# tqch/ddpm-torch

Hardware: AMD Instinct MI355X
Metric: training imgs/s/GPU + 1000-step DDPM samples/s, CIFAR-10 UNet @1/2/4/8 MI355X (higher is better)
Workload: dtype bf16; 1 GPU; configs/cifar10.json UNet (35.7M params), full Trainer.step, B=128 per GPU, 32x32, T=1000, dropout 0.1, Adam+clip+EMA; global_batch=128, rccl_ranks=1, parallelism=dp1

## Files before the change

### ddpm-torch_amd/csrc/common.h

```cpp
#pragma once
#include <hip/hip_runtime.h>
#include <stdint.h>

#define DDPM_OK 0
#define DDPM_ERR_SHAPE 1
#define DDPM_ERR_DTYPE 2
#define DDPM_ERR_ALIGN 3
#define DDPM_ERR_LAUNCH 4
#define DDPM_ERR_NULL 5

#define DDPM_F32 0
#define DDPM_BF16 1

typedef unsigned short bf16_t;

typedef float f32x4 __attribute__((ext_vector_type(4)));
typedef float f32x16 __attribute__((ext_vector_type(16)));
typedef short s16x8 __attribute__((ext_vector_type(8)));
typedef unsigned int u32x4 __attribute__((ext_vector_type(4)));

__device__ __forceinline__ float bf2f(bf16_t v) { return __uint_as_float(((unsigned)v) << 16); }
typedef __attribute__((ext_vector_type(2))) __bf16 hw_bf16x2;
typedef __attribute__((ext_vector_type(2))) float hw_f32x2;
__device__ __forceinline__ unsigned pack_bf2(float lo, float hi) {
    hw_f32x2 v; v.x = lo; v.y = hi;
    return __builtin_bit_cast(unsigned, __builtin_convertvector(v, hw_bf16x2));
}
__device__ __forceinline__ bf16_t f2bf(float f) { return (bf16_t)(pack_bf2(f, 0.f) & 0xffffu); }

template <typename T> struct Elem;
template <> struct Elem<float> {
    static constexpr int VEC = 4;
    __device__ static __forceinline__ float ld(const float* p) { return *p; }
    __device__ static __forceinline__ void st(float* p, float v) { *p = v; }
    __device__ static __forceinline__ void unpack(const u32x4& v, float* f) {
        f[0] = __uint_as_float(v.x); f[1] = __uint_as_float(v.y); f[2] = __uint_as_float(v.z); f[3] = __uint_as_float(v.w);
    }
    __device__ static __forceinline__ u32x4 pack(const float* f) {
        u32x4 v; v.x = __float_as_uint(f[0]); v.y = __float_as_uint(f[1]); v.z = __float_as_uint(f[2]); v.w = __float_as_uint(f[3]);
        return v;
    }
};
template <> struct Elem<bf16_t> {
    static constexpr int VEC = 8;
    __device__ static __forceinline__ float ld(const bf16_t* p) { return bf2f(*p); }
    __device__ static __forceinline__ void st(bf16_t* p, float v) { *p = f2bf(v); }
    __device__ static __forceinline__ void unpack(const u32x4& v, float* f) {
        f[0] = __uint_as_float(v.x << 16); f[1] = __uint_as_float(v.x & 0xffff0000u);
        f[2] = __uint_as_float(v.y << 16); f[3] = __uint_as_float(v.y & 0xffff0000u);
        f[4] = __uint_as_float(v.z << 16); f[5] = __uint_as_float(v.z & 0xffff0000u);
        f[6] = __uint_as_float(v.w << 16); f[7] = __uint_as_float(v.w & 0xffff0000u);
    }
    __device__ static __forceinline__ u32x4 pack(const float* f) {
        u32x4 v; v.x = pack_bf2(f[0], f[1]); v.y = pack_bf2(f[2], f[3]); v.z = pack_bf2(f[4], f[5]); v.w = pack_bf2(f[6], f[7]);
        return v;
    }
};

__device__ __forceinline__ u32x4 ldg16(const void* p) { return *reinterpret_cast<const u32x4*>(p); }
__device__ __forceinline__ void stg16(void* p, const u32x4& v) { *reinterpret_cast<u32x4*>(p) = v; }
__device__ __forceinline__ u32x4 zero16() { u32x4 v; v.x = v.y = v.z = v.w = 0u; return v; }

__device__ __forceinline__ float wave_sum(float v) {
#pragma unroll
    for (int o = 32; o > 0; o >>= 1) v += __shfl_xor(v, o, 64);
    return v;
}
__device__ __forceinline__ float wave_max(float v) {
#pragma unroll
    for (int o = 32; o > 0; o >>= 1) v = fmaxf(v, __shfl_xor(v, o, 64));
    return v;
}

__device__ __forceinline__ float sigmoidf_(float z) { return 1.0f / (1.0f + __expf(-z)); }
__device__ __forceinline__ float siluf_(float z) { return z * sigmoidf_(z); }
__device__ __forceinline__ float silu_fast_(float z) { return z * __builtin_amdgcn_rcpf(1.0f + __expf(-z)); }
__device__ __forceinline__ float silu_gradf_(float z) { float s = sigmoidf_(z); return s * (1.0f + z * (1.0f - s)); }

struct FastDiv {
    unsigned mul, shift, d;
};
__device__ __forceinline__ unsigned fdiv(unsigned n, const FastDiv& f) {
    return (unsigned)(((unsigned long long)n * f.mul) >> f.shift);
}
static inline FastDiv make_fastdiv(unsigned d) {
    FastDiv f; f.d = d ? d : 1; f.mul = 1u << 31; f.shift = 31;
    if (d <= 1) return f;
    unsigned l = 0; while ((1ull << l) < d) ++l;
    f.shift = 31 + l;
    if ((1ull << l) == d) return f;
    f.mul = (unsigned)((1ull << f.shift) / d + 1);
    return f;
}

__device__ __forceinline__ unsigned mix32(unsigned x) {
    x ^= x >> 16; x *= 0x7feb352dU; x ^= x >> 15; x *= 0x846ca68bU; x ^= x >> 16;
    return x;
}
__device__ __forceinline__ unsigned dropout_word(unsigned long long seed, unsigned long long pair) {
    const unsigned lo = (unsigned)pair, hi = (unsigned)(pair >> 32);
    return mix32(lo ^ mix32(hi + (unsigned)seed) ^ (unsigned)(seed >> 32) * 0x9E3779B9u);
}
__device__ __forceinline__ bool dropout_keep(unsigned long long seed, unsigned long long idx, unsigned thresh16) {
    const unsigned w = dropout_word(seed, idx >> 1);
    return ((idx & 1) ? (w >> 16) : (w & 0xffffu)) >= thresh16;
}
__device__ __forceinline__ unsigned dropout_h0(unsigned long long seed) {
    return mix32((unsigned)seed) ^ ((unsigned)(seed >> 32) * 0x9E3779B9u);
}
__device__ __forceinline__ unsigned dropout_word32(unsigned h0, unsigned pair) { return mix32(pair ^ h0); }
static inline unsigned dropout_thresh16(float p) {
    const double th = (double)p * 65536.0;
    return th <= 0 ? 0u : (th >= 65536.0 ? 65536u : (unsigned)(th + 0.5));
}
__device__ __forceinline__ float silu_grad_fast_(float z) {
    const float s = __builtin_amdgcn_rcpf(1.0f + __expf(-z));
    return s * (1.0f + z * (1.0f - s));
}

#include <atomic>
struct DevOnce {
    std::atomic<unsigned long long> mask{0};
    static unsigned long long bit() { int d = 0; (void)hipGetDevice(&d); return 1ull << (d & 63); }
    bool operator!() const { return !(mask.load(std::memory_order_acquire) & bit()); }
    DevOnce& operator=(bool) { mask.fetch_or(bit(), std::memory_order_release); return *this; }
};

static inline int check_launch() { return hipGetLastError() == hipSuccess ? DDPM_OK : DDPM_ERR_LAUNCH; }
static inline bool aligned16(const void* p) { return (((uintptr_t)p) & 15) == 0; }

int ddpm_sumsq_finish_launch(const float* partial, int n, float* total_sq, void* stream);
int ddpm_reserved_cus();
static inline int ddpm_cu_budget(int wanted) { const int left = 256 - ddpm_reserved_cus(); return wanted < left ? wanted : (left > 1 ? left : 1); }
int ddpm_pointwise_launch(const void* x, long long x_ld, const void* w, void* y, long long y_ld, const float* bias, const void* residual,
                          long long res_ld, int accumulate, int M, int N, int K, int dry, void* stream);
int ddpm_edgeconv_few_out_launch(const void* x, long long x_ld, const void* w, void* y, const float* bias, int B, int H, int W, int C, int N,
                                 int dry, void* stream);
int ddpm_edgeconv_few_in_launch(const void* x, long long x_ld, const void* w, void* y, long long y_ld, const float* bias, int B, int H, int W,
                                int C, int N, int dry, void* stream);
int ddpm_conv3x3_stream_launch(const void* x, long long x_ld, const void* w, void* y, long long y_ld, const float* bias, const float* rowbias,
                               long long rowbias_ld, const void* residual, long long res_ld, int accumulate, int B, int H, int W, int C, int N,
                               int upsample, int xcd, int dry, void* stream);
```

### ddpm-torch_amd/csrc/plan.hip

```cpp
#include "common.h"
#include "../../include/ddpm_hip.h"
#include "../../include/ddpm_hip_debug.h"

#include <cstring>
#include <mutex>
#include <type_traits>
#include <utility>
#include <vector>

namespace {

typedef unsigned long long word_t;

template <class T> inline T from_word(word_t w) {
    if constexpr (std::is_pointer<T>::value) {
        return reinterpret_cast<T>(static_cast<uintptr_t>(w));
    } else if constexpr (std::is_same<T, float>::value) {
        const unsigned u = static_cast<unsigned>(w);
        float f;
        std::memcpy(&f, &u, 4);
        return f;
    } else {
        return static_cast<T>(w);
    }
}

typedef int (*thunk_t)(const word_t*);

template <class... A, size_t... I> inline int invoke(int (*fn)(A...), const word_t* w, std::index_sequence<I...>) {
    return fn(from_word<A>(w[I])...);
}
template <class... A> constexpr int arity(int (*)(A...)) { return (int)sizeof...(A); }
template <class... A> inline int invoke_all(int (*fn)(A...), const word_t* w) { return invoke(fn, w, std::index_sequence_for<A...>{}); }

struct EntryPoint {
    const char* name;
    thunk_t thunk;
    int nargs;
};

#define EP(fn) {#fn, [](const word_t* w) -> int { return invoke_all(&fn, w); }, arity(&fn)}

}

extern "C" int ddpm_stream_order(void* waiter, void* signaller);
extern "C" int ddpm_fill_zero(void* p, long long bytes, void* stream);

namespace {

const EntryPoint kEntryPoints[] = {
    EP(ddpm_conv2d_nhwc), EP(ddpm_conv2d_wgrad_nhwc), EP(ddpm_conv3x3_wgrad_nhwc), EP(ddpm_conv3x3_wgrad_up_nhwc), EP(ddpm_conv1x1_wgrad_nhwc),
    EP(ddpm_wgrad_reduce), EP(ddpm_wgrad_unpack), EP(ddpm_wgrad_unpack_sumsq), EP(ddpm_gemm),
    EP(ddpm_attention_fwd), EP(ddpm_attention_fwd_lse), EP(ddpm_attention_bwd), EP(ddpm_groupnorm_silu_fwd),
    EP(ddpm_groupnorm_silu_bwd), EP(ddpm_timestep_embedding), EP(ddpm_nchw_to_nhwc), EP(ddpm_pack_weight), EP(ddpm_pack_weight_multi),
    EP(ddpm_q_sample), EP(ddpm_mse_fwd), EP(ddpm_mse_bwd), EP(ddpm_weighted_sum_f32), EP(ddpm_atb_f32), EP(ddpm_p_sample_step), EP(ddpm_vlb_terms), EP(ddpm_vlb_terms_bwd), EP(ddpm_gather_i64),
    EP(ddpm_add_i64), EP(ddpm_gather_rows_f32), EP(ddpm_silu_fwd), EP(ddpm_silu_bwd), EP(ddpm_colsum), EP(ddpm_upsample2x_bwd), EP(ddpm_resample2x_nhwc),
    EP(ddpm_add_rows), EP(ddpm_softmax_fwd), EP(ddpm_softmax_bwd), EP(ddpm_sumsq_accumulate), EP(ddpm_adam_ema_step), EP(ddpm_mt_grad_sumsq),
    EP(ddpm_mt_adam_ema), EP(ddpm_mt_gather_f32), EP(ddpm_mfma_probe), EP(ddpm_copy_probe), EP(ddpm_dropout_mask), EP(ddpm_stream_order), EP(ddpm_fill_zero),
    EP(ddpm_toy_time_table), EP(ddpm_toy_decoder_fwd), EP(ddpm_toy_decoder_bwd), EP(ddpm_toy_time_table_bwd),
    EP(ddpm_manifold_kth_f16), EP(ddpm_manifold_cover_f16),
};
constexpr int kNumEntryPoints = (int)(sizeof(kEntryPoints) / sizeof(kEntryPoints[0]));

struct Entry {
    thunk_t thunk;
    int first_word;
    int ep;
};

struct Plan {
    std::vector<Entry> entries;
    std::vector<word_t> words;
    std::vector<int> segment_end;
    int failed_index = -1;
    int failed_status = 0;
};

constexpr int kRing = 2048;
struct EventRing {
    hipEvent_t ev[kRing];
    unsigned next = 0;
    bool ready = false;
};
EventRing g_rings[64];
std::mutex g_ring_mutex;

}

extern "C" {

int ddpm_stream_order(void* waiter, void* signaller) {
    if (waiter == signaller) return DDPM_OK;
    int dev = 0;
    if (hipGetDevice(&dev) != hipSuccess) return DDPM_ERR_LAUNCH;
    EventRing& r = g_rings[dev & 63];
    hipEvent_t e;
    {
        std::lock_guard<std::mutex> lock(g_ring_mutex);
        if (!r.ready) {
            for (int i = 0; i < kRing; ++i)
                if (hipEventCreateWithFlags(&r.ev[i], hipEventDisableTiming) != hipSuccess) return DDPM_ERR_LAUNCH;
            r.ready = true;
        }
        e = r.ev[r.next++ % kRing];
    }
    if (hipEventRecord(e, (hipStream_t)signaller) != hipSuccess) return DDPM_ERR_LAUNCH;
    if (hipStreamWaitEvent((hipStream_t)waiter, e, 0) != hipSuccess) return DDPM_ERR_LAUNCH;
    return DDPM_OK;
}

int ddpm_fill_zero(void* p, long long bytes, void* stream) {
    if (bytes < 0) return DDPM_ERR_SHAPE;
    if (bytes == 0) return DDPM_OK;
    if (!p) return DDPM_ERR_NULL;
    return hipMemsetAsync(p, 0, (size_t)bytes, (hipStream_t)stream) == hipSuccess ? DDPM_OK : DDPM_ERR_LAUNCH;
}

void* ddpm_plan_create(void) { return new Plan(); }

int ddpm_plan_destroy(void* plan) {
    delete static_cast<Plan*>(plan);
    return DDPM_OK;
}

int ddpm_plan_append(void* plan, const char* entry, const unsigned long long* words, int n_words) {
    if (!plan || !entry || (!words && n_words > 0)) return -DDPM_ERR_NULL;
    Plan* p = static_cast<Plan*>(plan);
    for (int i = 0; i < kNumEntryPoints; ++i) {
        if (std::strcmp(kEntryPoints[i].name, entry) != 0) continue;
        if (kEntryPoints[i].nargs != n_words) return -DDPM_ERR_SHAPE;
        Entry e;
        e.thunk = kEntryPoints[i].thunk;
        e.first_word = (int)p->words.size();
        e.ep = i;
        p->words.insert(p->words.end(), words, words + n_words);
        p->entries.push_back(e);
        return (int)p->entries.size() - 1;
    }
    return -DDPM_ERR_SHAPE;
}

int ddpm_plan_cut(void* plan) {
    if (!plan) return -DDPM_ERR_NULL;
    Plan* p = static_cast<Plan*>(plan);
    p->segment_end.push_back((int)p->entries.size());
    return (int)p->segment_end.size() - 1;
}

int ddpm_plan_segments(void* plan) {
    if (!plan) return -DDPM_ERR_NULL;
    Plan* p = static_cast<Plan*>(plan);
    const int closed = (int)p->segment_end.size();
    const int last_end = closed ? p->segment_end.back() : 0;
    return closed + ((int)p->entries.size() > last_end ? 1 : 0);
}

int ddpm_plan_entries(void* plan) { return plan ? (int)static_cast<Plan*>(plan)->entries.size() : -DDPM_ERR_NULL; }

int ddpm_plan_run(void* plan, int segment) {
    if (!plan) return DDPM_ERR_NULL;
    Plan* p = static_cast<Plan*>(plan);
    const int closed = (int)p->segment_end.size();
    if (segment < 0 || segment > closed) return DDPM_ERR_SHAPE;
    const int first = segment ? p->segment_end[segment - 1] : 0;
    const int last = segment < closed ? p->segment_end[segment] : (int)p->entries.size();
    const word_t* words = p->words.data();
    const Entry* e = p->entries.data();
    for (int i = first; i < last; ++i) {
        const int rc = e[i].thunk(words + e[i].first_word);
        if (rc != DDPM_OK) {
            p->failed_index = i;
            p->failed_status = rc;
            return rc;
        }
    }
    return DDPM_OK;
}

const char* ddpm_plan_failed_entry(void* plan, int* index) {
    if (!plan) return nullptr;
    Plan* p = static_cast<Plan*>(plan);
    if (index) *index = p->failed_index;
    return p->failed_index < 0 ? nullptr : kEntryPoints[p->entries[p->failed_index].ep].name;
}

int ddpm_plan_entry_arity(const char* entry) {
    if (!entry) return -1;
    for (int i = 0; i < kNumEntryPoints; ++i)
        if (std::strcmp(kEntryPoints[i].name, entry) == 0) return kEntryPoints[i].nargs;
    return -1;
}

}
```

Baseline: 14160 imgs/s.

## Attach completion events to producer kernel launches and drop redundant stream waits

Adds a plan resolution pass that, for each cross-stream ordering entry, finds the last kernel launched on the signalling stream and marks it as producer. The producer's kernel is then launched with hipExtLaunchKernel carrying a stop event, so the waiter can call hipStreamWaitEvent on it directly instead of issuing a separate event record. Duplicate edges with no intervening work are skipped. This cuts host-side API calls and queue packets per step, at the cost of overriding hipLaunchKernelGGL globally and relying on the kernel's last argument being its stream.

Result: faster. 14360 imgs/s (median of 6 runs) (+1.4%).

```diff
diff --git a/ddpm-torch_amd/csrc/common.h b/ddpm-torch_amd/csrc/common.h
--- a/ddpm-torch_amd/csrc/common.h
+++ b/ddpm-torch_amd/csrc/common.h
@@ -1,5 +1,6 @@
 #pragma once
 #include <hip/hip_runtime.h>
+#include <hip/hip_ext.h>
 #include <stdint.h>
 
 #define DDPM_OK 0
@@ -126,6 +127,28 @@
     DevOnce& operator=(bool) { mask.fetch_or(bit(), std::memory_order_release); return *this; }
 };
 
+struct DdpmLaunchEdge {
+    hipStream_t stream = nullptr;
+    hipEvent_t event = nullptr;
+    bool armed = false;
+    bool attached = false;
+};
+extern thread_local DdpmLaunchEdge g_ddpm_launch_edge;
+
+template <class... P> static inline void ddpm_launch_with_event(DdpmLaunchEdge& edge, void (*kernel)(P...), dim3 grid, dim3 block, unsigned lds,
+                                                                hipStream_t st, P... formal) {
+    void* args[sizeof...(P) + 1] = {(void*)&formal..., nullptr};
+    if (hipExtLaunchKernel((const void*)kernel, grid, block, args, lds, st, nullptr, edge.event, 0) == hipSuccess) edge.attached = true;
+}
+template <class... P, class... A> static inline void ddpm_launch(void (*kernel)(P...), dim3 grid, dim3 block, unsigned lds, hipStream_t st, A&&... args) {
+    static_assert(sizeof...(P) == sizeof...(A), "kernel argument count");
+    DdpmLaunchEdge& edge = g_ddpm_launch_edge;
+    if (edge.armed && edge.stream == st) ddpm_launch_with_event<P...>(edge, kernel, grid, block, lds, st, static_cast<P>(args)...);
+    else kernel<<<grid, block, lds, st>>>(args...);
+}
+#undef hipLaunchKernelGGL
+#define hipLaunchKernelGGL(kernel, grid, block, lds, stream, ...) ddpm_launch(kernel, dim3(grid), dim3(block), (unsigned)(lds), stream, __VA_ARGS__)
+
 static inline int check_launch() { return hipGetLastError() == hipSuccess ? DDPM_OK : DDPM_ERR_LAUNCH; }
 static inline bool aligned16(const void* p) { return (((uintptr_t)p) & 15) == 0; }
 
diff --git a/ddpm-torch_amd/csrc/plan.hip b/ddpm-torch_amd/csrc/plan.hip
--- a/ddpm-torch_amd/csrc/plan.hip
+++ b/ddpm-torch_amd/csrc/plan.hip
@@ -33,13 +33,17 @@
 template <class... A> constexpr int arity(int (*)(A...)) { return (int)sizeof...(A); }
 template <class... A> inline int invoke_all(int (*fn)(A...), const word_t* w) { return invoke(fn, w, std::index_sequence_for<A...>{}); }
 
+enum EntryKind { EP_KERNELS, EP_ENQUEUES, EP_EDGE };
+
 struct EntryPoint {
     const char* name;
     thunk_t thunk;
     int nargs;
-};
-
-#define EP(fn) {#fn, [](const word_t* w) -> int { return invoke_all(&fn, w); }, arity(&fn)}
+    EntryKind kind;
+};
+
+#define EP(fn) {#fn, [](const word_t* w) -> int { return invoke_all(&fn, w); }, arity(&fn), EP_KERNELS}
+#define EP_AS(fn, kind) {#fn, [](const word_t* w) -> int { return invoke_all(&fn, w); }, arity(&fn), kind}
 
 }
 
@@ -56,22 +60,28 @@
     EP(ddpm_q_sample), EP(ddpm_mse_fwd), EP(ddpm_mse_bwd), EP(ddpm_weighted_sum_f32), EP(ddpm_atb_f32), EP(ddpm_p_sample_step), EP(ddpm_vlb_terms), EP(ddpm_vlb_terms_bwd), EP(ddpm_gather_i64),
     EP(ddpm_add_i64), EP(ddpm_gather_rows_f32), EP(ddpm_silu_fwd), EP(ddpm_silu_bwd), EP(ddpm_colsum), EP(ddpm_upsample2x_bwd), EP(ddpm_resample2x_nhwc),
     EP(ddpm_add_rows), EP(ddpm_softmax_fwd), EP(ddpm_softmax_bwd), EP(ddpm_sumsq_accumulate), EP(ddpm_adam_ema_step), EP(ddpm_mt_grad_sumsq),
-    EP(ddpm_mt_adam_ema), EP(ddpm_mt_gather_f32), EP(ddpm_mfma_probe), EP(ddpm_copy_probe), EP(ddpm_dropout_mask), EP(ddpm_stream_order), EP(ddpm_fill_zero),
+    EP(ddpm_mt_adam_ema), EP(ddpm_mt_gather_f32), EP(ddpm_mfma_probe), EP(ddpm_copy_probe), EP(ddpm_dropout_mask), EP_AS(ddpm_stream_order, EP_EDGE), EP_AS(ddpm_fill_zero, EP_ENQUEUES),
     EP(ddpm_toy_time_table), EP(ddpm_toy_decoder_fwd), EP(ddpm_toy_decoder_bwd), EP(ddpm_toy_time_table_bwd),
     EP(ddpm_manifold_kth_f16), EP(ddpm_manifold_cover_f16),
 };
 constexpr int kNumEntryPoints = (int)(sizeof(kEntryPoints) / sizeof(kEntryPoints[0]));
+
+enum Mode : unsigned char { RUN, PRODUCER, WAIT, RECORD, SKIP };
 
 struct Entry {
     thunk_t thunk;
     int first_word;
     int ep;
+    Mode mode = RUN;
+    int producer = -1;
 };
 
 struct Plan {
     std::vector<Entry> entries;
     std::vector<word_t> words;
     std::vector<int> segment_end;
+    std::vector<hipEvent_t> bound;
+    size_t resolved_entries = 0, resolved_cuts = 0;
     int failed_index = -1;
     int failed_status = 0;
 };
@@ -79,34 +89,76 @@
 constexpr int kRing = 2048;
 struct EventRing {
     hipEvent_t ev[kRing];
-    unsigned next = 0;
+    std::atomic<unsigned> next{0};
     bool ready = false;
 };
 EventRing g_rings[64];
 std::mutex g_ring_mutex;
 
-}
+EventRing* ring_of_device() {
+    int dev = 0;
+    if (hipGetDevice(&dev) != hipSuccess) return nullptr;
+    EventRing& r = g_rings[dev & 63];
+    std::lock_guard<std::mutex> lock(g_ring_mutex);
+    if (!r.ready) {
+        for (int i = 0; i < kRing; ++i)
+            if (hipEventCreateWithFlags(&r.ev[i], hipEventDisableTiming) != hipSuccess) return nullptr;
+        r.ready = true;
+    }
+    return &r;
+}
+inline hipEvent_t next_event(EventRing& r) { return r.ev[r.next.fetch_add(1, std::memory_order_relaxed) % kRing]; }
+
+inline int record_and_wait(EventRing& r, hipStream_t waiter, hipStream_t signaller) {
+    const hipEvent_t e = next_event(r);
+    if (hipEventRecord(e, signaller) != hipSuccess) return DDPM_ERR_LAUNCH;
+    if (hipStreamWaitEvent(waiter, e, 0) != hipSuccess) return DDPM_ERR_LAUNCH;
+    return DDPM_OK;
+}
+
+void resolve(Plan* p) {
+    const int n = (int)p->entries.size();
+    const word_t* words = p->words.data();
+    for (Entry& e : p->entries) { e.mode = RUN; e.producer = -1; }
+    size_t seg = 0;
+    int first = 0;
+    for (int i = 0; i < n; ++i) {
+        while (seg < p->segment_end.size() && p->segment_end[seg] <= i) first = p->segment_end[seg++];
+        Entry& e = p->entries[i];
+        if (kEntryPoints[e.ep].kind != EP_EDGE) continue;
+        const word_t waiter = words[e.first_word], signaller = words[e.first_word + 1];
+        if (waiter == signaller) continue;
+        e.mode = RECORD;
+        for (int j = i - 1; j >= first; --j) {
+            const Entry& q = p->entries[j];
+            const EntryPoint& ep = kEntryPoints[q.ep];
+            if (ep.kind == EP_EDGE) {
+                if (words[q.first_word] == waiter && words[q.first_word + 1] == signaller) { e.mode = SKIP; break; }
+                if (words[q.first_word] == signaller && words[q.first_word + 1] != signaller) break;
+                continue;
+            }
+            if (words[q.first_word + ep.nargs - 1] != signaller) continue;
+            if (ep.kind == EP_KERNELS) { e.mode = WAIT; e.producer = j; }
+            break;
+        }
+        if (e.mode == WAIT) p->entries[e.producer].mode = PRODUCER;
+    }
+    p->bound.assign(n, nullptr);
+    p->resolved_entries = p->entries.size();
+    p->resolved_cuts = p->segment_end.size();
+}
+
+}
+
+thread_local DdpmLaunchEdge g_ddpm_launch_edge;
 
 extern "C" {
 
 int ddpm_stream_order(void* waiter, void* signaller) {
     if (waiter == signaller) return DDPM_OK;
-    int dev = 0;
-    if (hipGetDevice(&dev) != hipSuccess) return DDPM_ERR_LAUNCH;
-    EventRing& r = g_rings[dev & 63];
-    hipEvent_t e;
-    {
-        std::lock_guard<std::mutex> lock(g_ring_mutex);
-        if (!r.ready) {
-            for (int i = 0; i < kRing; ++i)
-                if (hipEventCreateWithFlags(&r.ev[i], hipEventDisableTiming) != hipSuccess) return DDPM_ERR_LAUNCH;
-            r.ready = true;
-        }
-        e = r.ev[r.next++ % kRing];
-    }
-    if (hipEventRecord(e, (hipStream_t)signaller) != hipSuccess) return DDPM_ERR_LAUNCH;
-    if (hipStreamWaitEvent((hipStream_t)waiter, e, 0) != hipSuccess) return DDPM_ERR_LAUNCH;
-    return DDPM_OK;
+    EventRing* r = ring_of_device();
+    if (!r) return DDPM_ERR_LAUNCH;
+    return record_and_wait(*r, (hipStream_t)waiter, (hipStream_t)signaller);
 }
 
 int ddpm_fill_zero(void* p, long long bytes, void* stream) {
@@ -164,10 +216,35 @@
     if (segment < 0 || segment > closed) return DDPM_ERR_SHAPE;
     const int first = segment ? p->segment_end[segment - 1] : 0;
     const int last = segment < closed ? p->segment_end[segment] : (int)p->entries.size();
+    if (p->resolved_entries != p->entries.size() || p->resolved_cuts != p->segment_end.size()) resolve(p);
     const word_t* words = p->words.data();
     const Entry* e = p->entries.data();
+    EventRing* ring = nullptr;
+    DdpmLaunchEdge& arm = g_ddpm_launch_edge;
     for (int i = first; i < last; ++i) {
-        const int rc = e[i].thunk(words + e[i].first_word);
+        const word_t* w = words + e[i].first_word;
+        int rc = DDPM_OK;
+        if (e[i].mode == RUN) {
+            rc = e[i].thunk(w);
+        } else if (e[i].mode == SKIP) {
+            continue;
+        } else {
+            if (!ring && !(ring = ring_of_device())) rc = DDPM_ERR_LAUNCH;
+            else if (e[i].mode == PRODUCER) {
+                arm.stream = (hipStream_t)(uintptr_t)w[kEntryPoints[e[i].ep].nargs - 1];
+                arm.event = next_event(*ring);
+                arm.attached = false;
+                arm.armed = true;
+                rc = e[i].thunk(w);
+                arm.armed = false;
+                p->bound[i] = arm.attached ? arm.event : nullptr;
+            } else {
+                const hipStream_t waiter = (hipStream_t)(uintptr_t)w[0], signaller = (hipStream_t)(uintptr_t)w[1];
+                const hipEvent_t ev = e[i].mode == WAIT ? p->bound[e[i].producer] : nullptr;
+                if (ev) rc = hipStreamWaitEvent(waiter, ev, 0) == hipSuccess ? DDPM_OK : DDPM_ERR_LAUNCH;
+                else rc = record_and_wait(*ring, waiter, signaller);
+            }
+        }
         if (rc != DDPM_OK) {
             p->failed_index = i;
             p->failed_status = rc;
```
